# VITA-Group/SinNeRF

Hardware: NVIDIA H100
Metric: rays/sec (64c+64f samples, 8x256 MLP) (higher is better)
Workload: dtype fp32-parity: fp16 hi/lo split x3 on wgmma, fp32 accumulate

## Files before the change

### sinnerf_b200/csrc/field_tc.cu

```cuda
#include <stddef.h>
#include <stdlib.h>

#include <type_traits>
#include <utility>

#include "act16.cuh"
#include "common.cuh"
#include "wgmma.cuh"

namespace snb {
using namespace wg;

constexpr int kTile = 128;
constexpr int kNh = 128;
constexpr int kKc = 32;
constexpr uint32_t kStepBytes = kNh * 16 * 2;
constexpr int kWgs = 2;
constexpr int kThreads = (kWgs + 1) * 128;
constexpr int kProducerRegs = 24, kConsumerRegs = 240;
static_assert(128 * kProducerRegs + kWgs * 128 * kConsumerRegs <= 65536, "register file");
constexpr size_t kSmemOptIn = 232448;

enum { SRC_ENC = 0, SRC_HID = 1, SRC_DIR = 2 };

// ... 243 lines not shown
    double acc = k == kWidth ? (double)bd[n] : 0.0;
    for (int j = 0; j < kWidth; ++j) acc += (double)Wd[n * 283 + j] * (double)(k == kWidth ? bf[j] : Wf[j * kWidth + k]);
    if (k == kWidth) fused[kHalf * kWidth + n] = (float)acc;
    else fused[n * kWidth + k] = (float)acc;
  }
}

template <bool kBf16, bool kSplit>
__global__ void pack_tc_kernel(ParamPtrs pp, int precision, int new_activation, unsigned char* image, int only_if_dirty) {
  constexpr ConstLayout CL = make_const_layout();
  const ChunkTable& tab = c_chunks;
  PackedHeader* hdr = reinterpret_cast<PackedHeader*>(image);
  if (only_if_dirty && !hdr->dirty) return;
  float* cst = reinterpret_cast<float*>(image + sizeof(PackedHeader));
  unsigned char* chunks = image + sizeof(PackedHeader) + kConstBytes;
  const float* fused = reinterpret_cast<const float*>(chunks + chunks_bytes(precision));
  const int gtid = blockIdx.x * blockDim.x + threadIdx.x, gsz = gridDim.x * blockDim.x;
  if (gtid == 0) {
    hdr->magic = kMagic;
    hdr->precision = precision;
    hdr->new_activation = new_activation;
    hdr->cta_group = 1;
  }
  for (int e = gtid; e < kConstFloats; e += gsz) {
    float v = 0.f;
    if (e < CL.sigma_w) {
      int l = 0;
      while (l + 1 < kNumGemm && e >= CL.b[l + 1]) ++l;
      v = l == 9 ? fused[kHalf * kWidth + (e - CL.b[l])] : pp.p[param_weight_index(l) + 1][e - CL.b[l]];
    } else if (e < CL.sigma_b) v = pp.p[kSigmaW][e - CL.sigma_w];
    else if (e == CL.sigma_b) v = pp.p[kSigmaB][0];
    else if (e >= CL.rgb_w && e < CL.rgb_b) v = pp.p[kRgbW][e - CL.rgb_w];
    else if (e >= CL.rgb_b && e < CL.rgb_b + 3) v = pp.p[kRgbB][e - CL.rgb_b];
    cst[e] = v;
  }
  constexpr int kParts = kSplit ? 2 : 1;
  const int total = tab.steps_total * kNh * 16;
  for (int e = gtid; e < total; e += gsz) {
    const int gstep = e / (kNh * 16), rem = e - gstep * (kNh * 16);
    const int r = rem >> 4, k16 = rem & 15;
    int ci = 0;
    while (ci + 1 < tab.n_total && gstep >= tab.c[ci + 1].off) ++ci;
    const Chunk c = tab.c[ci];
    const int kk = (gstep - c.off) * 16 + k16;
    const int l = c.layer;
    const int n = c.half * kNh + r;
    const int kpad = c.w16 * 16 + kk;
    const int col = kpad < gemm_k(l) ? gemm_src_col(l, kpad) : -1;
    const int src_k = l == 0 ? 63 : (l == 4 ? 319 : (l == 9 ? 283 : 256));
    float w = col >= 0 ? pp.p[param_weight_index(l)][n * src_k + col] : 0.f;
    if (l == 9 && kpad < kWidth) w = fused[n * kWidth + kpad];
    const uint32_t part = kStepBytes * c.steps;
    unsigned char* base = chunks + (size_t)c.off * (kStepBytes * kParts);
    const uint32_t off = (uint32_t)(kk >> 3) * (kNh * 16) + r * 16 + (kk & 7) * 2;
    if (kSplit) {
      uint16_t hi, lo;
      split16<kBf16>(w, hi, lo);
      *reinterpret_cast<uint16_t*>(base + off) = hi;
      *reinterpret_cast<uint16_t*>(base + part + off) = lo;
    } else {
      if (!kBf16) w = fminf(fmaxf(w, -65504.f), 65504.f);
      *reinterpret_cast<uint16_t*>(base + off) = cvt16<kBf16>(w);
    }
  }
}

int launch_pack_tc(const float* const* params, int precision, int new_activation, void* image, int only_if_dirty,
                   cudaStream_t st) {
  ParamPtrs pp;
  for (int i = 0; i < SNB_N_PARAM_TENSORS; ++i) pp.p[i] = params[i];
  unsigned char* img = reinterpret_cast<unsigned char*>(image);
  if (precision < SNB_PREC_F16X3 || precision > SNB_PREC_F16)
    return fail(SNB_ERR_INVALID, "launch_pack_tc: precision %d is not a tensor-core mode", precision);
  float* fused = reinterpret_cast<float*>(img + sizeof(PackedHeader) + kConstBytes + chunks_bytes(precision));
  fuse_bottleneck_kernel<<<132, 256, 0, st>>>(pp, fused, reinterpret_cast<const PackedHeader*>(img), only_if_dirty);
  if (int rc = check_launch("fuse_bottleneck_kernel")) return rc;
  if (precision == SNB_PREC_F16X3) pack_tc_kernel<false, true><<<264, 256, 0, st>>>(pp, precision, new_activation, img, only_if_dirty);
  else if (precision == SNB_PREC_BF16X3) pack_tc_kernel<true, true><<<264, 256, 0, st>>>(pp, precision, new_activation, img, only_if_dirty);
  else if (precision == SNB_PREC_BF16) pack_tc_kernel<true, false><<<264, 256, 0, st>>>(pp, precision, new_activation, img, only_if_dirty);
  else pack_tc_kernel<false, false><<<264, 256, 0, st>>>(pp, precision, new_activation, img, only_if_dirty);
  return check_launch("pack_tc_kernel");
}

template <bool kSplit>
struct TcSmem {
  static constexpr int kParts = kSplit ? 2 : 1;
  static constexpr uint32_t kStageBytes = kStepBytes * (kKc / 16) * kParts;
  static constexpr size_t kActBytes = (size_t)kParts * kTile * (kWidth + kXyzPad) * 2;
  static constexpr int kStages = (int)((kSmemOptIn - 128 - kActBytes) / (kStageBytes + 2 * sizeof(uint64_t)));
  alignas(128) unsigned char ring[kStages][kStageBytes];
  alignas(128) unsigned char hid[kParts][kTile * kWidth * 2];
  alignas(128) unsigned char enc[kParts][kTile * kXyzPad * 2];
  uint64_t full[kStages], empty[kStages];
};
static_assert(kDirPad <= kXyzPad, "the direction encoding fits in the xyz encoding's buffer");
static_assert(sizeof(TcSmem<true>) + 128 <= kSmemOptIn && sizeof(TcSmem<false>) + 128 <= kSmemOptIn, "shared memory");
static_assert(TcSmem<true>::kStages >= 4 && TcSmem<false>::kStages >= 6, "weight ring depth");

struct TcParams {
  const unsigned char* image;
  const float* rays;
  const float* z;
  int n_samples;
  const float* x;
  long long x_stride;
  long long n_points;
  int sigma_only;
  float* out;
  float* save_enc;
  float* save_dir;
  float* save_h;
  float* save_g;
  unsigned char* a_enc;
  unsigned char* a_dir;
  unsigned char* a_h;
  unsigned char* a_g;
  uint32_t* a_mask;
  long long ppad;
};

template <bool kBf16, bool kSplit, bool kEmbedded, int kTrain = 0>
__global__ void __launch_bounds__(kThreads, 1) field_tc_kernel(TcParams p) {
  static_assert(!(kTrain != 0 && kEmbedded), "the training forward is the fused (rays, z) entry only");
  using Smem = TcSmem<kSplit>;
  extern __shared__ unsigned char smem_raw[];
  Smem& s = *reinterpret_cast<Smem*>((reinterpret_cast<uintptr_t>(smem_raw) + 127) & ~uintptr_t(127));
  constexpr ConstLayout CL = make_const_layout();
  constexpr int kStages = Smem::kStages;
  constexpr int kParts = Smem::kParts;
  const ChunkTable& tab = c_chunks;
  const int tid = threadIdx.x, warp = tid >> 5, lane = tid & 31;
  const PackedHeader* hdr = reinterpret_cast<const PackedHeader*>(p.image);
  const int new_activation = hdr->new_activation;
  const float* g_cst = reinterpret_cast<const float*>(p.image + sizeof(PackedHeader));
  const unsigned char* g_chunks = p.image + sizeof(PackedHeader) + kConstBytes;
  const long long ntiles = (p.n_points + kTile - 1) / kTile;
  const int n_chunks = p.sigma_only ? tab.n_sigma_only : tab.n_total;

  if (tid == 0) {
    for (int i = 0; i < kStages; ++i) { mbar_init(&s.full[i], 1); mbar_init(&s.empty[i], kWgs * 4); }
    fence_mbar_init();
  }
  __syncthreads();

  if (warp >= kWgs * 4) {
    setmaxnreg_dec<kProducerRegs>();
    if (warp == kWgs * 4 && elect_one()) {
      const long long my_tiles = ntiles > (long long)blockIdx.x ? (ntiles - 1 - blockIdx.x) / gridDim.x + 1 : 0;
      const long long n_loads = my_tiles * n_chunks;
      uint32_t st = 0, ph = 0;
      int ci = 0;
      for (long long i = 0; i < n_loads; ++i) {
        mbar_wait(&s.empty[st], ph ^ 1);
        const Chunk c = tab.c[ci];
        const uint32_t bytes = kStepBytes * kParts * c.steps;
        mbar_arrive_expect_tx(&s.full[st], bytes);
        bulk_g2s(s.ring[st], g_chunks + (size_t)c.off * (kStepBytes * kParts), bytes, &s.full[st]);
        if (++ci == n_chunks) ci = 0;
        if (++st == kStages) { st = 0; ph ^= 1; }
      }
    }
    return;
  }
  setmaxnreg_inc<kConsumerRegs>();

  const int wgi = warp >> 2, wq = warp & 3, tq = lane & 3;
  const int r0 = wgi * 64 + wq * 16 + (lane >> 2);
  auto wg_sync = [&]() { named_bar_sync(1 + wgi, 128); };
  constexpr uint32_t kHidPart = kTile * kWidth * 2, kEncPart = kTile * kXyzPad * 2;
  constexpr uint32_t kOffRing = offsetof(Smem, ring), kOffHid = offsetof(Smem, hid), kOffEnc = offsetof(Smem, enc);
  const uint32_t sbase = smem_u32(&s);
  const uint32_t a_wg = sbase + wgi * 64 * 16;
  const uint32_t hid_thr = sbase + kOffHid + r0 * 16 + tq * 4;
  const int er = wgi * 64 + (tid & 63), epart = (tid >> 6) & 1;

  auto store_cell16 = [&](unsigned char* base, long long pt, int f8, int F, const float (&v)[8]) SNB_INLINE {
    if (pt >= p.ppad) return;
    const bool live = pt < p.n_points;
    uint4 c;
    c.x = live ? pack_half2_sat(v[0], v[1]) : 0u; c.y = live ? pack_half2_sat(v[2], v[3]) : 0u;
    c.z = live ? pack_half2_sat(v[4], v[5]) : 0u; c.w = live ? pack_half2_sat(v[6], v[7]) : 0u;
    *reinterpret_cast<uint4*>(base + a16_cell(pt, f8, F)) = c;
  };

  struct RowIn { float4 q0, q1; float z; };
  RowIn in{};
  auto load_row = [&](long long tile) SNB_INLINE {
    const long long pt = tile * kTile + er;
    if (!kEmbedded && tile < ntiles && pt < p.n_points) {
      const long long ray = pt / p.n_samples;
      in.q0 = *reinterpret_cast<const float4*>(p.rays + ray * 8);
      in.q1 = *reinterpret_cast<const float4*>(p.rays + ray * 8 + 4);
      in.z = p.z[pt];
    }
  };
  auto encode = [&](auto ltag, auto ptag, long long tile) SNB_INLINE {
    constexpr int L = decltype(ltag)::value, P = decltype(ptag)::value;
    constexpr bool kXyz = L == SNB_XYZ_FREQS;
    constexpr int kCh = 3 * (2 * L + 1), kPad = (kCh + 7) / 8 * 8, kK8 = kPad / 16;
    constexpr int c_lo = 8 * kK8 * P, c_hi = 8 * kK8 * (P + 1);
    const long long pt = tile * kTile + er;
    const bool live = pt < p.n_points;
    float v[kPad];
#pragma unroll
    for (int j = 0; j < kPad; ++j) v[j] = 0.f;
    if (kEmbedded) {
      const float* xr = p.x + pt * p.x_stride;
      const int nin = p.sigma_only ? kXyzCh : kXyzCh + kDirCh;
#pragma unroll
      for (int j = c_lo; j < (c_hi < kCh ? c_hi : kCh); ++j) {
        const int col = kXyz ? j : kXyzCh + j;
        v[j] = (live && col < nin) ? xr[col] : 0.f;
      }
    } else {
      float x[3] = {0.f, 0.f, 0.f};
      if (live) {
        if (kXyz) {
          x[0] = __fadd_rn(in.q0.x, __fmul_rn(in.q0.w, in.z));
          x[1] = __fadd_rn(in.q0.y, __fmul_rn(in.q1.x, in.z));
          x[2] = __fadd_rn(in.q0.z, __fmul_rn(in.q1.y, in.z));
        } else {
          x[0] = in.q0.w; x[1] = in.q1.x; x[2] = in.q1.y;
        }
      }
      v[0] = x[0]; v[1] = x[1]; v[2] = x[2];
#pragma unroll
      for (int f = 0; f < L; ++f)
#pragma unroll
        for (int c = 0; c < 3; ++c) {
          const int cs = 3 + 6 * f + c, cc = cs + 3;
          if ((cs >= c_lo && cs < c_hi) || (cc >= c_lo && cc < c_hi)) {
            float sn, cs_;
            if (kSplit) sincosf(x[c] * (float)(1 << f), &sn, &cs_);
            else sincos_fast(x[c] * (float)(1 << f), &sn, &cs_);
            v[cs] = sn;
            v[cc] = cs_;
          }
        }
    }
    static_for<kK8>([&](auto ktag) SNB_INLINE {
      constexpr int k8 = kK8 * P + decltype(ktag)::value;
      const float v8[8] = {v[8 * k8], v[8 * k8 + 1], v[8 * k8 + 2], v[8 * k8 + 3], v[8 * k8 + 4], v[8 * k8 + 5], v[8 * k8 + 6], v[8 * k8 + 7]};
      if (!kEmbedded) {
        if (kTrain == 1 && live) {
          float4* dst = reinterpret_cast<float4*>((kXyz ? p.save_enc + pt * kXyzPad : p.save_dir + pt * kDirPad) + k8 * 8);
          dst[0] = make_float4(v8[0], v8[1], v8[2], v8[3]); dst[1] = make_float4(v8[4], v8[5], v8[6], v8[7]);
        }
        if (kTrain == 2) store_cell16(kXyz ? p.a_enc : p.a_dir, pt, k8, kXyz ? kXyzPad : kDirPad, v8);
      }
      uint32_t h[4], l[4];
#pragma unroll
      for (int j = 0; j < 4; ++j) split_pair<kBf16, kSplit>(v8[2 * j], v8[2 * j + 1], h[j], l[j]);
      const uint32_t a = sbase + kOffEnc + k8 * (kTile * 16) + er * 16;
      st_shared_v4(a, h[0], h[1], h[2], h[3]);
      if (kSplit) st_shared_v4(a + kEncPart, l[0], l[1], l[2], l[3]);
    });
  };
  auto encode_rows = [&](auto ltag, long long tile) SNB_INLINE {
    if (epart == 0) encode(ltag, std::integral_constant<int, 0>{}, tile);
    else encode(ltag, std::integral_constant<int, 1>{}, tile);
  };

  auto mma = [&](float (&d)[64], uint64_t a, uint64_t b, bool first) SNB_INLINE {
    if (first) {
      if (kBf16) wgmma_m64n128_bf16_first(d, a, b);
      else wgmma_m64n128_f16_first(d, a, b);
    } else {
      if (kBf16) wgmma_m64n128_bf16(d, a, b, 1u);
      else wgmma_m64n128_f16(d, a, b, 1u);
    }
  };
  auto issue_step = [&](float (&d)[64], uint32_t ah, uint32_t al, uint32_t bh, uint32_t bl, bool first) SNB_INLINE {
    const uint64_t da_h = make_smem_desc(ah, kTile * 16, 128), db_h = make_smem_desc(bh, kNh * 16, 128);
    mma(d, da_h, db_h, first);
    if (kSplit) {
      mma(d, make_smem_desc(al, kTile * 16, 128), db_h, false);
      mma(d, da_h, make_smem_desc(bl, kNh * 16, 128), false);
    }
  };

  constexpr bool kDrained = kTrain != 0;
  float acc[2][64];
  float sig[2] = {0.f, 0.f};

  uint32_t st = 0, ph = 0;
  auto prev_stage = [&]() { return st == 0 ? (uint32_t)kStages - 1 : st - 1; };
  auto issue = [&](auto ctag) SNB_INLINE {
    constexpr int ci = decltype(ctag)::value;
    constexpr Chunk c = h_chunks.c[ci];
    float (&d)[64] = acc[c.half];
    mbar_wait(&s.full[st], ph);
    wgmma_fence();
    const uint32_t bh = sbase + kOffRing + st * Smem::kStageBytes, bl = bh + kStepBytes * c.steps;
    uint32_t abase;
    asm volatile("mov.b32 %0, %1;" : "=r"(abase) : "r"(a_wg));
    const uint32_t ah = abase + (c.src == SRC_HID ? kOffHid : kOffEnc) + c.a16 * 2 * (kTile * 16);
    constexpr uint32_t part = c.src == SRC_HID ? kHidPart : kEncPart;
    static_for<c.steps>([&](auto ktag) SNB_INLINE {
      constexpr int ks = decltype(ktag)::value;
      issue_step(d, ah + ks * 2 * (kTile * 16), ah + ks * 2 * (kTile * 16) + part, bh + ks * kStepBytes,
                 bl + ks * kStepBytes, ks == 0 && c.first);
    });
    wgmma_commit();
    if (kDrained ? !(c.first && c.half == 0) : ci != 0) {
      wgmma_wait<1>();
      if (lane == 0) mbar_arrive(&s.empty[prev_stage()]);
      __syncwarp();
    }
    if (++st == kStages) { st = 0; ph ^= 1; }
  };
  auto issue_range = [&](auto c0tag, auto ntag) SNB_INLINE {
    static_for<decltype(ntag)::value>([&](auto i) SNB_INLINE { issue(Int<decltype(c0tag)::value + decltype(i)::value>{}); });
  };
  auto drain = [&]() {
    wgmma_wait<0>();
    if (lane == 0) mbar_arrive(&s.empty[prev_stage()]);
    __syncwarp();
  };

  struct Block16 { uint32_t h16[4][2], mask[2]; };
  auto epi_block = [&](auto sigtag, auto htag, auto btag, int l, long long pt0) SNB_INLINE {
    constexpr bool kSigma = decltype(sigtag)::value;
    constexpr int h = decltype(htag)::value, b = decltype(btag)::value;
    const float* bias = g_cst + l * kWidth;
    const float (&d)[64] = acc[h];
    Block16 k16{};
    if (kSigma && h == 0 && b == 0) { sig[0] = 0.f; sig[1] = 0.f; }
    static_for<4>([&](auto jtag) SNB_INLINE {
      constexpr int jj = decltype(jtag)::value, j = 4 * b + jj;
      const int col = h * kNh + 8 * j + 2 * tq;
      const float2 bb = ldg_f2_here(bias + col);
#pragma unroll
      for (int rr = 0; rr < 2; ++rr) {
        float x0 = d[4 * j + 2 * rr] + bb.x, x1 = d[4 * j + 2 * rr + 1] + bb.y;
        uint32_t hi, lo;
        if (kTrain == 0 && !kSigma) {
          split_pair_relu<kBf16, kSplit>(x0, x1, hi, lo);
        } else {
          x0 = fmaxf(x0, 0.f); x1 = fmaxf(x1, 0.f);
          if (kSigma) {
            const float2 ww = ldg_f2_here(g_cst + CL.sigma_w + col);
            sig[rr] = fmaf(x0, ww.x, sig[rr]); sig[rr] = fmaf(x1, ww.y, sig[rr]);
          }
          split_pair<kBf16, kSplit, true>(x0, x1, hi, lo);
          const long long pt = pt0 + 8 * rr;
          if (kTrain == 1 && pt < p.n_points)
            *reinterpret_cast<float2*>(p.save_h + ((size_t)l * p.n_points + pt) * kWidth + col) = make_float2(x0, x1);
          if (kTrain == 2) {
            k16.h16[jj][rr] = kBf16 ? pack_half2_sat(x0, x1) : hi;
            k16.mask[rr] |= ((x0 > 0.f ? 1u : 0u) << (col & 31)) | ((x1 > 0.f ? 1u : 0u) << ((col & 31) + 1));
          }
        }
        const uint32_t a = hid_thr + (h * 16 + j) * (kTile * 16) + rr * 128;
        st_shared_u32(a, hi);
        if (kSplit) st_shared_u32(a + kHidPart, lo);
      }
    });
    if (kTrain == 2) {
#pragma unroll
      for (int rr = 0; rr < 2; ++rr) {
        k16.mask[rr] |= __shfl_xor_sync(0xffffffffu, k16.mask[rr], 1);
        k16.mask[rr] |= __shfl_xor_sync(0xffffffffu, k16.mask[rr], 2);
      }
    }
    return k16;
  };
  auto epi_half_end = [&]() SNB_INLINE {
    fence_proxy_async_smem();
    wg_sync();
  };
  auto sigma_head = [&](long long pt0) SNB_INLINE {
#pragma unroll
    for (int rr = 0; rr < 2; ++rr) {
      float v = sig[rr];
      v += __shfl_xor_sync(0xffffffffu, v, 1);
      v += __shfl_xor_sync(0xffffffffu, v, 2);
      sig[rr] = v + __ldg(g_cst + CL.sigma_b);
      const long long pt = pt0 + 8 * rr;
      if (p.sigma_only && tq == 0 && pt < p.n_points) p.out[pt] = sig[rr];
    }
  };

  auto dir_epilogue = [&](const float (&d)[64], long long pt0) SNB_INLINE {
    const float sh = new_activation ? 1.0f : 0.0f;
    float a[2][3] = {{0.f, 0.f, 0.f}, {0.f, 0.f, 0.f}};
#pragma unroll
    for (int j = 0; j < 16; ++j) {
      const int col = 8 * j + 2 * tq;
      const float2 bb = __ldg(reinterpret_cast<const float2*>(g_cst + CL.b[9] + col));
      const float2 w0 = __ldg(reinterpret_cast<const float2*>(g_cst + CL.rgb_w + col));
      const float2 w1 = __ldg(reinterpret_cast<const float2*>(g_cst + CL.rgb_w + kHalf + col));
      const float2 w2 = __ldg(reinterpret_cast<const float2*>(g_cst + CL.rgb_w + 2 * kHalf + col));
#pragma unroll
      for (int rr = 0; rr < 2; ++rr) {
        const long long pt = pt0 + 8 * rr;
        float x0 = d[4 * j + 2 * rr] + (bb.x - sh), x1 = d[4 * j + 2 * rr + 1] + (bb.y - sh);
        if (new_activation) { x0 = softplus_fast(x0); x1 = softplus_fast(x1); }
        else { x0 = fmaxf(x0, 0.f); x1 = fmaxf(x1, 0.f); }
        if (kTrain == 1 && pt < p.n_points) *reinterpret_cast<float2*>(p.save_g + pt * kHalf + col) = make_float2(x0, x1);
        if (kTrain == 2 && pt < p.ppad)
          *reinterpret_cast<uint32_t*>(p.a_g + a16_cell(pt, col >> 3, kHalf) + (col & 7) * 2) =
              pt < p.n_points ? pack_half2_sat(x0, x1) : 0u;
        a[rr][0] = fmaf(x1, w0.y, fmaf(x0, w0.x, a[rr][0]));
        a[rr][1] = fmaf(x1, w1.y, fmaf(x0, w1.x, a[rr][1]));
        a[rr][2] = fmaf(x1, w2.y, fmaf(x0, w2.x, a[rr][2]));
      }
    }
#pragma unroll
    for (int rr = 0; rr < 2; ++rr) {
      float c[3];
#pragma unroll
      for (int k = 0; k < 3; ++k) {
        float v = a[rr][k];
        v += __shfl_xor_sync(0xffffffffu, v, 1);
        v += __shfl_xor_sync(0xffffffffu, v, 2);
        v += __ldg(g_cst + CL.rgb_b + k);
        c[k] = new_activation ? widened_sigmoid_f(v) : sigmoid_f(v);
      }
      const long long pt = pt0 + 8 * rr;
      if (tq == 0 && pt < p.n_points) reinterpret_cast<float4*>(p.out)[pt] = make_float4(c[0], c[1], c[2], sig[rr]);
    }
  };

  auto trunk_epilogue = [&](auto ltag, int l, long long tile, long long pt0) SNB_INLINE {
    constexpr int L = decltype(ltag)::value;
    Block16 k16[2][4];
    static_for<2>([&](auto htag) SNB_INLINE {
      static_for<4>([&](auto btag) SNB_INLINE {
        k16[decltype(htag)::value][decltype(btag)::value] = epi_block(std::bool_constant<L == 7>{}, htag, btag, l, pt0);
      });
    });
    if (L == 7) sigma_head(pt0);
    if (L == 4 && !p.sigma_only) encode_rows(Int<SNB_DIR_FREQS>{}, tile);
    epi_half_end();
    if (kTrain == 2) {
      unsigned char* hb = p.a_h + (size_t)l * (size_t)p.ppad * (kWidth * 2);
#pragma unroll
      for (int rr = 0; rr < 2; ++rr) {
        const long long pt = pt0 + 8 * rr;
        if (pt >= p.ppad) continue;
        const bool live = pt < p.n_points;
#pragma unroll
        for (int h = 0; h < 2; ++h) {
#pragma unroll
          for (int j = 0; j < 16; ++j) {
            const int col = h * kNh + 8 * j + 2 * tq;
            *reinterpret_cast<uint32_t*>(hb + a16_cell(pt, col >> 3, kWidth) + (col & 7) * 2) =
                live ? k16[h][j / 4].h16[j % 4][rr] : 0u;
          }
#pragma unroll
          for (int b = 0; b < 4; ++b)
            if (tq == 0) p.a_mask[a16_mask_index(l, h * 4 + b, pt, p.ppad)] = live ? k16[h][b].mask[rr] : 0u;
        }
      }
    }
  };

  auto trunk_layer = [&](auto ltag, int l, long long tile, long long pt0) SNB_INLINE {
    constexpr int L = decltype(ltag)::value;
    constexpr int c0 = chunk_index(L, 0), n0 = chunk_count(L, 0), c1 = chunk_index(L, 1), n1 = chunk_count(L, 1);
    constexpr int e = enc_chunks(L);
    if constexpr (kDrained) {
      issue_range(Int<c0>{}, Int<n0>{});
      issue_range(Int<c1>{}, Int<n1>{});
      drain();
      trunk_epilogue(ltag, l, tile, pt0);
    } else if constexpr (L == 0) {
      issue_range(Int<c0>{}, Int<n0>{});
      static_for<4>([&](auto btag) SNB_INLINE {
        constexpr int b = decltype(btag)::value;
        if constexpr (b < n1) issue(Int<c1 + b>{});
        epi_block(std::false_type{}, Int<0>{}, btag, 0, pt0);
      });
      epi_half_end();
      wgmma_wait<0>();
    } else {
      static_for<4>([&](auto btag) SNB_INLINE {
        issue(Int<c0 + decltype(btag)::value>{});
        epi_block(std::false_type{}, Int<1>{}, btag, l - 1, pt0);
      });
      epi_half_end();
      issue_range(Int<c0 + 4>{}, Int<n0 - 4>{});
      issue_range(Int<c1>{}, Int<e + 1>{});
      static_for<4>([&](auto btag) SNB_INLINE {
        issue(Int<c1 + e + 1 + decltype(btag)::value>{});
        epi_block(std::bool_constant<L == 7>{}, Int<0>{}, btag, l, pt0);
      });
      if (L == 4 && !p.sigma_only) encode_rows(Int<SNB_DIR_FREQS>{}, tile);
      epi_half_end();
      issue_range(Int<c1 + e + 5>{}, Int<n1 - e - 5>{});
      if constexpr (L != 7) wgmma_wait<0>();
    }
  };
  auto tile_end = [&](long long tile, long long pt0) SNB_INLINE {
    constexpr int c9 = chunk_index(9, 0), n9 = chunk_count(9, 0);
    load_row(tile + gridDim.x);
    if (p.sigma_only) {
      if constexpr (!kDrained) {
        drain();
        static_for<4>([&](auto btag) SNB_INLINE { epi_block(std::true_type{}, Int<1>{}, btag, 7, pt0); });
        sigma_head(pt0);
        epi_half_end();
      }
      return;
    }
    if constexpr (kDrained) {
      issue_range(Int<c9>{}, Int<n9>{});
    } else {
      static_for<4>([&](auto btag) SNB_INLINE {
        issue(Int<c9 + decltype(btag)::value>{});
        epi_block(std::true_type{}, Int<1>{}, btag, 7, pt0);
      });
      sigma_head(pt0);
      epi_half_end();
      issue_range(Int<c9 + 4>{}, Int<n9 - 4>{});
    }
    drain();
    dir_epilogue(acc[0], pt0);
  };

  load_row(blockIdx.x);
  for (long long tile = blockIdx.x; tile < ntiles; tile += gridDim.x) {
    const long long pt0 = tile * kTile + r0;
    encode_rows(Int<SNB_XYZ_FREQS>{}, tile);
    fence_proxy_async_smem();
    wg_sync();
    trunk_layer(Int<0>{}, 0, tile, pt0);
#pragma unroll 1
    for (int l = 1; l < 4; ++l) trunk_layer(Int<1>{}, l, tile, pt0);
    trunk_layer(Int<4>{}, 4, tile, pt0);
#pragma unroll 1
    for (int l = 5; l < 7; ++l) trunk_layer(Int<1>{}, l, tile, pt0);
    trunk_layer(Int<7>{}, 7, tile, pt0);
    tile_end(tile, pt0);
  }
}

template <bool kBf16, bool kSplit, bool kEmbedded, int kTrain = 0>
static int launch_tc(const TcParams& p, cudaStream_t st) {
  static SmemOptIn optin;
  const long long ntiles = (p.n_points + kTile - 1) / kTile;
  if (ntiles == 0) return SNB_OK;
  const size_t smem = sizeof(TcSmem<kSplit>) + 128;
  auto kern = field_tc_kernel<kBf16, kSplit, kEmbedded, kTrain>;
  if (int rc = ensure_smem(kern, optin, (int)smem, "field_tc")) return rc;
  long long ctas = sm_count();
  if (ctas > ntiles) ctas = ntiles;
  kern<<<(unsigned)ctas, kThreads, smem, st>>>(p);
  return check_launch("field_tc_kernel");
}

template <bool kEmbedded, int kTrain = 0>
static int dispatch_tc(int precision, const TcParams& p, cudaStream_t st) {
  switch (precision) {
    case SNB_PREC_F16X3: return launch_tc<false, true, kEmbedded, kTrain>(p, st);
    case SNB_PREC_BF16X3: return launch_tc<true, true, kEmbedded, kTrain>(p, st);
    case SNB_PREC_BF16: return launch_tc<true, false, kEmbedded, kTrain>(p, st);
    case SNB_PREC_F16: return launch_tc<false, false, kEmbedded, kTrain>(p, st);
  }
  return fail(SNB_ERR_INVALID, "precision %d is not a tensor-core mode", precision);
}

int field_forward_tc(const void* packed, int precision, const float* rays, const float* z, int64_t n_rays,
                     int n_samples, int sigma_only, float* raw, cudaStream_t st) {
  TcParams p{};
  p.image = reinterpret_cast<const unsigned char*>(packed);
  p.rays = rays; p.z = z; p.n_samples = n_samples;
  p.n_points = (long long)n_rays * n_samples;
  p.sigma_only = sigma_only;
  p.out = raw;
  return dispatch_tc<false>(precision, p, st);
}

int field_forward_train_tc(const void* packed, int precision, const float* rays, const float* z, int64_t n_rays,
                           int n_samples, int sigma_only, float* raw, float* save_enc, float* save_dir, float* save_h,
                           float* save_g, cudaStream_t st) {
  TcParams p{};
  p.image = reinterpret_cast<const unsigned char*>(packed);
  p.rays = rays; p.z = z; p.n_samples = n_samples;
  p.n_points = (long long)n_rays * n_samples;
  p.sigma_only = sigma_only;
  p.out = raw;
  p.save_enc = save_enc; p.save_dir = save_dir; p.save_h = save_h; p.save_g = save_g;
  return dispatch_tc<false, 1>(precision, p, st);
}

int field_forward_train16_tc(const void* packed, int precision, const float* rays, const float* z, int64_t n_rays,
                             int n_samples, int sigma_only, float* raw, void* act16, cudaStream_t st) {
  TcParams p{};
  p.image = reinterpret_cast<const unsigned char*>(packed);
  p.rays = rays; p.z = z; p.n_samples = n_samples;
  p.n_points = (long long)n_rays * n_samples;
  p.sigma_only = sigma_only;
  p.out = raw;
  const Act16Layout L = make_act16_layout(p.n_points);
  unsigned char* b = reinterpret_cast<unsigned char*>(act16);
  p.a_enc = b + L.enc; p.a_dir = b + L.dir; p.a_h = b + L.h[0]; p.a_g = b + L.g;
  p.a_mask = reinterpret_cast<uint32_t*>(b + L.mask);
  p.ppad = a16_pad(p.n_points);
  return dispatch_tc<false, 2>(precision, p, st);
}

int mlp_forward_tc(const void* packed, int precision, const float* x, int64_t x_stride, int64_t n_points,
                   int sigma_only, float* out, cudaStream_t st) {
  TcParams p{};
  p.image = reinterpret_cast<const unsigned char*>(packed);
  p.x = x; p.x_stride = x_stride;
  p.n_points = n_points;
  p.sigma_only = sigma_only;
  p.out = out;
  return dispatch_tc<true>(precision, p, st);
}

}
```

### sinnerf_b200/csrc/wgmma.cuh

```cuda
#pragma once
#include <cuda_fp16.h>
#include <cuda_bf16.h>
#include <stdint.h>

namespace snb {
namespace wg {

__device__ __forceinline__ uint32_t smem_u32(const void* p) { return (uint32_t)__cvta_generic_to_shared(p); }

__device__ __forceinline__ bool elect_one() {
  uint32_t pred = 0;
  asm volatile(
      "{\n\t.reg .pred p;\n\t"
      "elect.sync _|p, 0xffffffff;\n\t"
      "selp.u32 %0, 1, 0, p;\n\t}"
      : "=r"(pred));
  return pred != 0;
}

__device__ __forceinline__ void mbar_init(uint64_t* bar, uint32_t count) {
  asm volatile("mbarrier.init.shared::cta.b64 [%0], %1;" ::"r"(smem_u32(bar)), "r"(count));
}
__device__ __forceinline__ void fence_mbar_init() { asm volatile("fence.mbarrier_init.release.cluster;" ::: "memory"); }
__device__ __forceinline__ void mbar_arrive(uint64_t* bar) {
// ... 120 lines not shown
      "{%0, %1, %2, %3, %4, %5, %6, %7, %8, %9, %10, %11, %12, %13, %14, %15, %16, %17, %18, %19, %20, %21, %22, %23, %24, %25, %26, %27, %28, %29, %30, %31, %32, %33, %34, %35, %36, %37, %38, %39, %40, %41, %42, %43, %44, %45, %46, %47, %48, %49, %50, %51, %52, %53, %54, %55, %56, %57, %58, %59, %60, %61, %62, %63}, %64, %65, p, 1, 1, 1, 1;\n\t}"
      : "+f"(d[0]), "+f"(d[1]), "+f"(d[2]), "+f"(d[3]), "+f"(d[4]), "+f"(d[5]), "+f"(d[6]), "+f"(d[7]), "+f"(d[8]), "+f"(d[9]), "+f"(d[10]), "+f"(d[11]), "+f"(d[12]), "+f"(d[13]), "+f"(d[14]), "+f"(d[15]), "+f"(d[16]), "+f"(d[17]), "+f"(d[18]), "+f"(d[19]), "+f"(d[20]), "+f"(d[21]), "+f"(d[22]), "+f"(d[23]), "+f"(d[24]), "+f"(d[25]), "+f"(d[26]), "+f"(d[27]), "+f"(d[28]), "+f"(d[29]), "+f"(d[30]), "+f"(d[31]), "+f"(d[32]), "+f"(d[33]), "+f"(d[34]), "+f"(d[35]), "+f"(d[36]), "+f"(d[37]), "+f"(d[38]), "+f"(d[39]), "+f"(d[40]), "+f"(d[41]), "+f"(d[42]), "+f"(d[43]), "+f"(d[44]), "+f"(d[45]), "+f"(d[46]), "+f"(d[47]), "+f"(d[48]), "+f"(d[49]), "+f"(d[50]), "+f"(d[51]), "+f"(d[52]), "+f"(d[53]), "+f"(d[54]), "+f"(d[55]), "+f"(d[56]), "+f"(d[57]), "+f"(d[58]), "+f"(d[59]), "+f"(d[60]), "+f"(d[61]), "+f"(d[62]), "+f"(d[63])
      : "l"(a_desc), "l"(b_desc), "r"(accumulate)
      : "memory");
}

__device__ __forceinline__ void wgmma_m64n64_f16_mn(float (&d)[32], uint64_t a_desc, uint64_t b_desc, uint32_t accumulate) {
  asm volatile(
      "{\n\t.reg .pred p;\n\t"
      "setp.ne.b32 p, %34, 0;\n\t"
      "wgmma.mma_async.sync.aligned.m64n64k16.f32.f16.f16 "
      "{%0, %1, %2, %3, %4, %5, %6, %7, %8, %9, %10, %11, %12, %13, %14, %15, %16, %17, %18, %19, %20, %21, %22, %23, %24, %25, %26, %27, %28, %29, %30, %31}, %32, %33, p, 1, 1, 1, 1;\n\t}"
      : "+f"(d[0]), "+f"(d[1]), "+f"(d[2]), "+f"(d[3]), "+f"(d[4]), "+f"(d[5]), "+f"(d[6]), "+f"(d[7]), "+f"(d[8]), "+f"(d[9]), "+f"(d[10]), "+f"(d[11]), "+f"(d[12]), "+f"(d[13]), "+f"(d[14]), "+f"(d[15]), "+f"(d[16]), "+f"(d[17]), "+f"(d[18]), "+f"(d[19]), "+f"(d[20]), "+f"(d[21]), "+f"(d[22]), "+f"(d[23]), "+f"(d[24]), "+f"(d[25]), "+f"(d[26]), "+f"(d[27]), "+f"(d[28]), "+f"(d[29]), "+f"(d[30]), "+f"(d[31])
      : "l"(a_desc), "l"(b_desc), "r"(accumulate)
      : "memory");
}

__device__ __forceinline__ void wgmma_m64n32_f16_mn(float (&d)[16], uint64_t a_desc, uint64_t b_desc, uint32_t accumulate) {
  asm volatile(
      "{\n\t.reg .pred p;\n\t"
      "setp.ne.b32 p, %18, 0;\n\t"
      "wgmma.mma_async.sync.aligned.m64n32k16.f32.f16.f16 "
      "{%0, %1, %2, %3, %4, %5, %6, %7, %8, %9, %10, %11, %12, %13, %14, %15}, %16, %17, p, 1, 1, 1, 1;\n\t}"
      : "+f"(d[0]), "+f"(d[1]), "+f"(d[2]), "+f"(d[3]), "+f"(d[4]), "+f"(d[5]), "+f"(d[6]), "+f"(d[7]), "+f"(d[8]), "+f"(d[9]), "+f"(d[10]), "+f"(d[11]), "+f"(d[12]), "+f"(d[13]), "+f"(d[14]), "+f"(d[15])
      : "l"(a_desc), "l"(b_desc), "r"(accumulate)
      : "memory");
}

__device__ __forceinline__ void wgmma_m64n128_f16_rs(float (&d)[64], const uint32_t (&a)[4], uint64_t b_desc, uint32_t accumulate) {
  asm volatile(
      "{\n\t.reg .pred p;\n\t"
      "setp.ne.b32 p, %69, 0;\n\t"
      "wgmma.mma_async.sync.aligned.m64n128k16.f32.f16.f16 "
      "{%0, %1, %2, %3, %4, %5, %6, %7, %8, %9, %10, %11, %12, %13, %14, %15, %16, %17, %18, %19, %20, %21, %22, %23, %24, %25, %26, %27, %28, %29, %30, %31, %32, %33, %34, %35, %36, %37, %38, %39, %40, %41, %42, %43, %44, %45, %46, %47, %48, %49, %50, %51, %52, %53, %54, %55, %56, %57, %58, %59, %60, %61, %62, %63}, {%64, %65, %66, %67}, %68, p, 1, 1, 0;\n\t}"
      : "+f"(d[0]), "+f"(d[1]), "+f"(d[2]), "+f"(d[3]), "+f"(d[4]), "+f"(d[5]), "+f"(d[6]), "+f"(d[7]), "+f"(d[8]), "+f"(d[9]), "+f"(d[10]), "+f"(d[11]), "+f"(d[12]), "+f"(d[13]), "+f"(d[14]), "+f"(d[15]), "+f"(d[16]), "+f"(d[17]), "+f"(d[18]), "+f"(d[19]), "+f"(d[20]), "+f"(d[21]), "+f"(d[22]), "+f"(d[23]), "+f"(d[24]), "+f"(d[25]), "+f"(d[26]), "+f"(d[27]), "+f"(d[28]), "+f"(d[29]), "+f"(d[30]), "+f"(d[31]), "+f"(d[32]), "+f"(d[33]), "+f"(d[34]), "+f"(d[35]), "+f"(d[36]), "+f"(d[37]), "+f"(d[38]), "+f"(d[39]), "+f"(d[40]), "+f"(d[41]), "+f"(d[42]), "+f"(d[43]), "+f"(d[44]), "+f"(d[45]), "+f"(d[46]), "+f"(d[47]), "+f"(d[48]), "+f"(d[49]), "+f"(d[50]), "+f"(d[51]), "+f"(d[52]), "+f"(d[53]), "+f"(d[54]), "+f"(d[55]), "+f"(d[56]), "+f"(d[57]), "+f"(d[58]), "+f"(d[59]), "+f"(d[60]), "+f"(d[61]), "+f"(d[62]), "+f"(d[63])
      : "r"(a[0]), "r"(a[1]), "r"(a[2]), "r"(a[3]), "l"(b_desc), "r"(accumulate)
      : "memory");
}

__device__ __forceinline__ void wgmma_m64n256_bf16_mn(float (&d)[128], uint64_t a_desc, uint64_t b_desc, uint32_t accumulate) {
  asm volatile(
      "{\n\t.reg .pred p;\n\t"
      "setp.ne.b32 p, %130, 0;\n\t"
      "wgmma.mma_async.sync.aligned.m64n256k16.f32.bf16.bf16 "
      "{%0, %1, %2, %3, %4, %5, %6, %7, %8, %9, %10, %11, %12, %13, %14, %15, %16, %17, %18, %19, %20, %21, %22, %23, %24, %25, %26, %27, %28, %29, %30, %31, %32, %33, %34, %35, %36, %37, %38, %39, %40, %41, %42, %43, %44, %45, %46, %47, %48, %49, %50, %51, %52, %53, %54, %55, %56, %57, %58, %59, %60, %61, %62, %63, %64, %65, %66, %67, %68, %69, %70, %71, %72, %73, %74, %75, %76, %77, %78, %79, %80, %81, %82, %83, %84, %85, %86, %87, %88, %89, %90, %91, %92, %93, %94, %95, %96, %97, %98, %99, %100, %101, %102, %103, %104, %105, %106, %107, %108, %109, %110, %111, %112, %113, %114, %115, %116, %117, %118, %119, %120, %121, %122, %123, %124, %125, %126, %127}, %128, %129, p, 1, 1, 1, 1;\n\t}"
      : "+f"(d[0]), "+f"(d[1]), "+f"(d[2]), "+f"(d[3]), "+f"(d[4]), "+f"(d[5]), "+f"(d[6]), "+f"(d[7]), "+f"(d[8]), "+f"(d[9]), "+f"(d[10]), "+f"(d[11]), "+f"(d[12]), "+f"(d[13]), "+f"(d[14]), "+f"(d[15]), "+f"(d[16]), "+f"(d[17]), "+f"(d[18]), "+f"(d[19]), "+f"(d[20]), "+f"(d[21]), "+f"(d[22]), "+f"(d[23]), "+f"(d[24]), "+f"(d[25]), "+f"(d[26]), "+f"(d[27]), "+f"(d[28]), "+f"(d[29]), "+f"(d[30]), "+f"(d[31]), "+f"(d[32]), "+f"(d[33]), "+f"(d[34]), "+f"(d[35]), "+f"(d[36]), "+f"(d[37]), "+f"(d[38]), "+f"(d[39]), "+f"(d[40]), "+f"(d[41]), "+f"(d[42]), "+f"(d[43]), "+f"(d[44]), "+f"(d[45]), "+f"(d[46]), "+f"(d[47]), "+f"(d[48]), "+f"(d[49]), "+f"(d[50]), "+f"(d[51]), "+f"(d[52]), "+f"(d[53]), "+f"(d[54]), "+f"(d[55]), "+f"(d[56]), "+f"(d[57]), "+f"(d[58]), "+f"(d[59]), "+f"(d[60]), "+f"(d[61]), "+f"(d[62]), "+f"(d[63]), "+f"(d[64]), "+f"(d[65]), "+f"(d[66]), "+f"(d[67]), "+f"(d[68]), "+f"(d[69]), "+f"(d[70]), "+f"(d[71]), "+f"(d[72]), "+f"(d[73]), "+f"(d[74]), "+f"(d[75]), "+f"(d[76]), "+f"(d[77]), "+f"(d[78]), "+f"(d[79]), "+f"(d[80]), "+f"(d[81]), "+f"(d[82]), "+f"(d[83]), "+f"(d[84]), "+f"(d[85]), "+f"(d[86]), "+f"(d[87]), "+f"(d[88]), "+f"(d[89]), "+f"(d[90]), "+f"(d[91]), "+f"(d[92]), "+f"(d[93]), "+f"(d[94]), "+f"(d[95]), "+f"(d[96]), "+f"(d[97]), "+f"(d[98]), "+f"(d[99]), "+f"(d[100]), "+f"(d[101]), "+f"(d[102]), "+f"(d[103]), "+f"(d[104]), "+f"(d[105]), "+f"(d[106]), "+f"(d[107]), "+f"(d[108]), "+f"(d[109]), "+f"(d[110]), "+f"(d[111]), "+f"(d[112]), "+f"(d[113]), "+f"(d[114]), "+f"(d[115]), "+f"(d[116]), "+f"(d[117]), "+f"(d[118]), "+f"(d[119]), "+f"(d[120]), "+f"(d[121]), "+f"(d[122]), "+f"(d[123]), "+f"(d[124]), "+f"(d[125]), "+f"(d[126]), "+f"(d[127])
      : "l"(a_desc), "l"(b_desc), "r"(accumulate)
      : "memory");
}

__device__ __forceinline__ void wgmma_m64n64_bf16_mn(float (&d)[32], uint64_t a_desc, uint64_t b_desc, uint32_t accumulate) {
  asm volatile(
      "{\n\t.reg .pred p;\n\t"
      "setp.ne.b32 p, %34, 0;\n\t"
      "wgmma.mma_async.sync.aligned.m64n64k16.f32.bf16.bf16 "
      "{%0, %1, %2, %3, %4, %5, %6, %7, %8, %9, %10, %11, %12, %13, %14, %15, %16, %17, %18, %19, %20, %21, %22, %23, %24, %25, %26, %27, %28, %29, %30, %31}, %32, %33, p, 1, 1, 1, 1;\n\t}"
      : "+f"(d[0]), "+f"(d[1]), "+f"(d[2]), "+f"(d[3]), "+f"(d[4]), "+f"(d[5]), "+f"(d[6]), "+f"(d[7]), "+f"(d[8]), "+f"(d[9]), "+f"(d[10]), "+f"(d[11]), "+f"(d[12]), "+f"(d[13]), "+f"(d[14]), "+f"(d[15]), "+f"(d[16]), "+f"(d[17]), "+f"(d[18]), "+f"(d[19]), "+f"(d[20]), "+f"(d[21]), "+f"(d[22]), "+f"(d[23]), "+f"(d[24]), "+f"(d[25]), "+f"(d[26]), "+f"(d[27]), "+f"(d[28]), "+f"(d[29]), "+f"(d[30]), "+f"(d[31])
      : "l"(a_desc), "l"(b_desc), "r"(accumulate)
      : "memory");
}

__device__ __forceinline__ void wgmma_m64n32_bf16_mn(float (&d)[16], uint64_t a_desc, uint64_t b_desc, uint32_t accumulate) {
  asm volatile(
      "{\n\t.reg .pred p;\n\t"
      "setp.ne.b32 p, %18, 0;\n\t"
      "wgmma.mma_async.sync.aligned.m64n32k16.f32.bf16.bf16 "
      "{%0, %1, %2, %3, %4, %5, %6, %7, %8, %9, %10, %11, %12, %13, %14, %15}, %16, %17, p, 1, 1, 1, 1;\n\t}"
      : "+f"(d[0]), "+f"(d[1]), "+f"(d[2]), "+f"(d[3]), "+f"(d[4]), "+f"(d[5]), "+f"(d[6]), "+f"(d[7]), "+f"(d[8]), "+f"(d[9]), "+f"(d[10]), "+f"(d[11]), "+f"(d[12]), "+f"(d[13]), "+f"(d[14]), "+f"(d[15])
      : "l"(a_desc), "l"(b_desc), "r"(accumulate)
      : "memory");
}

__device__ __forceinline__ void wgmma_m64n128_bf16_rs(float (&d)[64], const uint32_t (&a)[4], uint64_t b_desc, uint32_t accumulate) {
  asm volatile(
      "{\n\t.reg .pred p;\n\t"
      "setp.ne.b32 p, %69, 0;\n\t"
      "wgmma.mma_async.sync.aligned.m64n128k16.f32.bf16.bf16 "
      "{%0, %1, %2, %3, %4, %5, %6, %7, %8, %9, %10, %11, %12, %13, %14, %15, %16, %17, %18, %19, %20, %21, %22, %23, %24, %25, %26, %27, %28, %29, %30, %31, %32, %33, %34, %35, %36, %37, %38, %39, %40, %41, %42, %43, %44, %45, %46, %47, %48, %49, %50, %51, %52, %53, %54, %55, %56, %57, %58, %59, %60, %61, %62, %63}, {%64, %65, %66, %67}, %68, p, 1, 1, 0;\n\t}"
      : "+f"(d[0]), "+f"(d[1]), "+f"(d[2]), "+f"(d[3]), "+f"(d[4]), "+f"(d[5]), "+f"(d[6]), "+f"(d[7]), "+f"(d[8]), "+f"(d[9]), "+f"(d[10]), "+f"(d[11]), "+f"(d[12]), "+f"(d[13]), "+f"(d[14]), "+f"(d[15]), "+f"(d[16]), "+f"(d[17]), "+f"(d[18]), "+f"(d[19]), "+f"(d[20]), "+f"(d[21]), "+f"(d[22]), "+f"(d[23]), "+f"(d[24]), "+f"(d[25]), "+f"(d[26]), "+f"(d[27]), "+f"(d[28]), "+f"(d[29]), "+f"(d[30]), "+f"(d[31]), "+f"(d[32]), "+f"(d[33]), "+f"(d[34]), "+f"(d[35]), "+f"(d[36]), "+f"(d[37]), "+f"(d[38]), "+f"(d[39]), "+f"(d[40]), "+f"(d[41]), "+f"(d[42]), "+f"(d[43]), "+f"(d[44]), "+f"(d[45]), "+f"(d[46]), "+f"(d[47]), "+f"(d[48]), "+f"(d[49]), "+f"(d[50]), "+f"(d[51]), "+f"(d[52]), "+f"(d[53]), "+f"(d[54]), "+f"(d[55]), "+f"(d[56]), "+f"(d[57]), "+f"(d[58]), "+f"(d[59]), "+f"(d[60]), "+f"(d[61]), "+f"(d[62]), "+f"(d[63])
      : "r"(a[0]), "r"(a[1]), "r"(a[2]), "r"(a[3]), "l"(b_desc), "r"(accumulate)
      : "memory");
}

}
}
```

Before: 1.139 million.

## Keep hidden-activation hi fragments in registers and feed wgmma from registers

In the inference path, the hi half of each hidden activation is now kept in registers (ahi[16][4]) and fed to register-sourced wgmma, instead of being written to shared memory. Only the lo part still goes to shared memory. The freed shared memory deepens the weight ring (4 to 8 stages for split mode), and some warpgroup syncs and fences are skipped when hidden data no longer passes through smem. The direction input is reloaded from global memory instead of being held across tiles. The risk is higher register pressure: 64 extra registers per thread on top of two 64-float accumulators, within a 240-register budget, which could cause spills.

```diff
diff --git a/sinnerf_b200/csrc/field_tc.cu b/sinnerf_b200/csrc/field_tc.cu
--- a/sinnerf_b200/csrc/field_tc.cu
+++ b/sinnerf_b200/csrc/field_tc.cu
@@ -349,20 +349,26 @@
   return check_launch("pack_tc_kernel");
 }
 
-template <bool kSplit>
+template <bool kSplit, bool kHiRegs>
 struct TcSmem {
   static constexpr int kParts = kSplit ? 2 : 1;
+  static constexpr int kHidParts = kHiRegs ? kParts - 1 : kParts;
   static constexpr uint32_t kStageBytes = kStepBytes * (kKc / 16) * kParts;
-  static constexpr size_t kActBytes = (size_t)kParts * kTile * (kWidth + kXyzPad) * 2;
+  static constexpr size_t kHidBytes = kHidParts ? (size_t)kHidParts * kTile * kWidth * 2 : 128;
+  static constexpr size_t kActBytes = kHidBytes + (size_t)kParts * kTile * kXyzPad * 2;
   static constexpr int kStages = (int)((kSmemOptIn - 128 - kActBytes) / (kStageBytes + 2 * sizeof(uint64_t)));
   alignas(128) unsigned char ring[kStages][kStageBytes];
-  alignas(128) unsigned char hid[kParts][kTile * kWidth * 2];
+  alignas(128) unsigned char hid[kHidBytes];
   alignas(128) unsigned char enc[kParts][kTile * kXyzPad * 2];
   uint64_t full[kStages], empty[kStages];
 };
+__host__ __device__ constexpr bool hi_in_regs(int train) { return train == 0; }
 static_assert(kDirPad <= kXyzPad, "the direction encoding fits in the xyz encoding's buffer");
-static_assert(sizeof(TcSmem<true>) + 128 <= kSmemOptIn && sizeof(TcSmem<false>) + 128 <= kSmemOptIn, "shared memory");
-static_assert(TcSmem<true>::kStages >= 4 && TcSmem<false>::kStages >= 6, "weight ring depth");
+static_assert(sizeof(TcSmem<true, false>) + 128 <= kSmemOptIn && sizeof(TcSmem<false, false>) + 128 <= kSmemOptIn &&
+              sizeof(TcSmem<true, true>) + 128 <= kSmemOptIn && sizeof(TcSmem<false, true>) + 128 <= kSmemOptIn,
+              "shared memory");
+static_assert(TcSmem<true, false>::kStages == 4 && TcSmem<false, false>::kStages == 18 &&
+              TcSmem<true, true>::kStages == 8 && TcSmem<false, true>::kStages == 26, "weight ring depth");
 
 struct TcParams {
   const unsigned char* image;
@@ -389,7 +395,8 @@
 template <bool kBf16, bool kSplit, bool kEmbedded, int kTrain = 0>
 __global__ void __launch_bounds__(kThreads, 1) field_tc_kernel(TcParams p) {
   static_assert(!(kTrain != 0 && kEmbedded), "the training forward is the fused (rays, z) entry only");
-  using Smem = TcSmem<kSplit>;
+  using Smem = TcSmem<kSplit, hi_in_regs(kTrain)>;
+  constexpr bool kHiRegs = hi_in_regs(kTrain);
   extern __shared__ unsigned char smem_raw[];
   Smem& s = *reinterpret_cast<Smem*>((reinterpret_cast<uintptr_t>(smem_raw) + 127) & ~uintptr_t(127));
   constexpr ConstLayout CL = make_const_layout();
@@ -435,6 +442,7 @@
   const int r0 = wgi * 64 + wq * 16 + (lane >> 2);
   auto wg_sync = [&]() { named_bar_sync(1 + wgi, 128); };
   constexpr uint32_t kHidPart = kTile * kWidth * 2, kEncPart = kTile * kXyzPad * 2;
+  constexpr uint32_t kHidLo = kHiRegs ? 0u : kHidPart;
   constexpr uint32_t kOffRing = offsetof(Smem, ring), kOffHid = offsetof(Smem, hid), kOffEnc = offsetof(Smem, enc);
   const uint32_t sbase = smem_u32(&s);
   const uint32_t a_wg = sbase + wgi * 64 * 16;
@@ -454,6 +462,7 @@
   RowIn in{};
   auto load_row = [&](long long tile) SNB_INLINE {
     const long long pt = tile * kTile + er;
+    if constexpr (kHiRegs) in = RowIn{};
     if (!kEmbedded && tile < ntiles && pt < p.n_points) {
       const long long ray = pt / p.n_samples;
       in.q0 = *reinterpret_cast<const float4*>(p.rays + ray * 8);
@@ -486,6 +495,9 @@
           x[0] = __fadd_rn(in.q0.x, __fmul_rn(in.q0.w, in.z));
           x[1] = __fadd_rn(in.q0.y, __fmul_rn(in.q1.x, in.z));
           x[2] = __fadd_rn(in.q0.z, __fmul_rn(in.q1.y, in.z));
+        } else if constexpr (kHiRegs) {
+          const float* d = p.rays + (pt / p.n_samples) * 8 + 3;
+          x[0] = d[0]; x[1] = d[1]; x[2] = d[2];
         } else {
           x[0] = in.q0.w; x[1] = in.q1.x; x[2] = in.q1.y;
         }
@@ -537,6 +549,15 @@
       else wgmma_m64n128_f16(d, a, b, 1u);
     }
   };
+  auto mma_rs = [&](float (&d)[64], const uint32_t (&a)[4], uint64_t b, bool first) SNB_INLINE {
+    if (first) {
+      if (kBf16) wgmma_m64n128_bf16_rs_first(d, a, b);
+      else wgmma_m64n128_f16_rs_first(d, a, b);
+    } else {
+      if (kBf16) wgmma_m64n128_bf16_rs(d, a, b, 1u);
+      else wgmma_m64n128_f16_rs(d, a, b, 1u);
+    }
+  };
   auto issue_step = [&](float (&d)[64], uint32_t ah, uint32_t al, uint32_t bh, uint32_t bl, bool first) SNB_INLINE {
     const uint64_t da_h = make_smem_desc(ah, kTile * 16, 128), db_h = make_smem_desc(bh, kNh * 16, 128);
     mma(d, da_h, db_h, first);
@@ -549,6 +570,7 @@
   constexpr bool kDrained = kTrain != 0;
   float acc[2][64];
   float sig[2] = {0.f, 0.f};
+  uint32_t ahi[16][4];
 
   uint32_t st = 0, ph = 0;
   auto prev_stage = [&]() { return st == 0 ? (uint32_t)kStages - 1 : st - 1; };
@@ -562,12 +584,24 @@
     uint32_t abase;
     asm volatile("mov.b32 %0, %1;" : "=r"(abase) : "r"(a_wg));
     const uint32_t ah = abase + (c.src == SRC_HID ? kOffHid : kOffEnc) + c.a16 * 2 * (kTile * 16);
-    constexpr uint32_t part = c.src == SRC_HID ? kHidPart : kEncPart;
-    static_for<c.steps>([&](auto ktag) SNB_INLINE {
-      constexpr int ks = decltype(ktag)::value;
-      issue_step(d, ah + ks * 2 * (kTile * 16), ah + ks * 2 * (kTile * 16) + part, bh + ks * kStepBytes,
-                 bl + ks * kStepBytes, ks == 0 && c.first);
-    });
+    if constexpr (kHiRegs && c.src == SRC_HID) {
+      static_for<c.steps>([&](auto ktag) SNB_INLINE {
+        constexpr int ks = decltype(ktag)::value;
+        const uint64_t db_h = make_smem_desc(bh + ks * kStepBytes, kNh * 16, 128);
+        mma_rs(d, ahi[c.a16 + ks], db_h, ks == 0 && c.first);
+        if (kSplit) {
+          mma(d, make_smem_desc(ah + ks * 2 * (kTile * 16), kTile * 16, 128), db_h, false);
+          mma_rs(d, ahi[c.a16 + ks], make_smem_desc(bl + ks * kStepBytes, kNh * 16, 128), false);
+        }
+      });
+    } else {
+      constexpr uint32_t part = c.src == SRC_HID ? kHidPart : kEncPart;
+      static_for<c.steps>([&](auto ktag) SNB_INLINE {
+        constexpr int ks = decltype(ktag)::value;
+        issue_step(d, ah + ks * 2 * (kTile * 16), ah + ks * 2 * (kTile * 16) + part, bh + ks * kStepBytes,
+                   bl + ks * kStepBytes, ks == 0 && c.first);
+      });
+    }
     wgmma_commit();
     if (kDrained ? !(c.first && c.half == 0) : ci != 0) {
       wgmma_wait<1>();
@@ -619,8 +653,9 @@
           }
         }
         const uint32_t a = hid_thr + (h * 16 + j) * (kTile * 16) + rr * 128;
-        st_shared_u32(a, hi);
-        if (kSplit) st_shared_u32(a + kHidPart, lo);
+        if constexpr (kHiRegs) ahi[8 * h + j / 2][(jj & 1) * 2 + rr] = hi;
+        else st_shared_u32(a, hi);
+        if (kSplit) st_shared_u32(a + kHidLo, lo);
       }
     });
     if (kTrain == 2) {
@@ -632,9 +667,11 @@
     }
     return k16;
   };
-  auto epi_half_end = [&]() SNB_INLINE {
-    fence_proxy_async_smem();
-    wg_sync();
+  auto epi_half_end = [&](auto enctag) SNB_INLINE {
+    if constexpr (kSplit || !kHiRegs || decltype(enctag)::value) {
+      fence_proxy_async_smem();
+      wg_sync();
+    }
   };
   auto sigma_head = [&](long long pt0) SNB_INLINE {
 #pragma unroll
@@ -699,7 +736,7 @@
     });
     if (L == 7) sigma_head(pt0);
     if (L == 4 && !p.sigma_only) encode_rows(Int<SNB_DIR_FREQS>{}, tile);
-    epi_half_end();
+    epi_half_end(std::bool_constant<L == 4>{});
     if (kTrain == 2) {
       unsigned char* hb = p.a_h + (size_t)l * (size_t)p.ppad * (kWidth * 2);
 #pragma unroll
@@ -739,14 +776,14 @@
         if constexpr (b < n1) issue(Int<c1 + b>{});
         epi_block(std::false_type{}, Int<0>{}, btag, 0, pt0);
       });
-      epi_half_end();
+      epi_half_end(std::false_type{});
       wgmma_wait<0>();
     } else {
       static_for<4>([&](auto btag) SNB_INLINE {
         issue(Int<c0 + decltype(btag)::value>{});
         epi_block(std::false_type{}, Int<1>{}, btag, l - 1, pt0);
       });
-      epi_half_end();
+      epi_half_end(std::false_type{});
       issue_range(Int<c0 + 4>{}, Int<n0 - 4>{});
       issue_range(Int<c1>{}, Int<e + 1>{});
       static_for<4>([&](auto btag) SNB_INLINE {
@@ -754,20 +791,21 @@
         epi_block(std::bool_constant<L == 7>{}, Int<0>{}, btag, l, pt0);
       });
       if (L == 4 && !p.sigma_only) encode_rows(Int<SNB_DIR_FREQS>{}, tile);
-      epi_half_end();
+      epi_half_end(std::bool_constant<L == 4>{});
       issue_range(Int<c1 + e + 5>{}, Int<n1 - e - 5>{});
       if constexpr (L != 7) wgmma_wait<0>();
     }
   };
   auto tile_end = [&](long long tile, long long pt0) SNB_INLINE {
     constexpr int c9 = chunk_index(9, 0), n9 = chunk_count(9, 0);
-    load_row(tile + gridDim.x);
+    if constexpr (!kHiRegs) load_row(tile + gridDim.x);
     if (p.sigma_only) {
       if constexpr (!kDrained) {
+        load_row(tile + gridDim.x);
         drain();
         static_for<4>([&](auto btag) SNB_INLINE { epi_block(std::true_type{}, Int<1>{}, btag, 7, pt0); });
         sigma_head(pt0);
-        epi_half_end();
+        epi_half_end(std::false_type{});
       }
       return;
     }
@@ -779,8 +817,9 @@
         epi_block(std::true_type{}, Int<1>{}, btag, 7, pt0);
       });
       sigma_head(pt0);
-      epi_half_end();
+      epi_half_end(std::false_type{});
       issue_range(Int<c9 + 4>{}, Int<n9 - 4>{});
+      load_row(tile + gridDim.x);
     }
     drain();
     dir_epilogue(acc[0], pt0);
@@ -808,7 +847,7 @@
   static SmemOptIn optin;
   const long long ntiles = (p.n_points + kTile - 1) / kTile;
   if (ntiles == 0) return SNB_OK;
-  const size_t smem = sizeof(TcSmem<kSplit>) + 128;
+  const size_t smem = sizeof(TcSmem<kSplit, hi_in_regs(kTrain)>) + 128;
   auto kern = field_tc_kernel<kBf16, kSplit, kEmbedded, kTrain>;
   if (int rc = ensure_smem(kern, optin, (int)smem, "field_tc")) return rc;
   long long ctas = sm_count();
diff --git a/sinnerf_b200/csrc/wgmma.cuh b/sinnerf_b200/csrc/wgmma.cuh
--- a/sinnerf_b200/csrc/wgmma.cuh
+++ b/sinnerf_b200/csrc/wgmma.cuh
@@ -226,5 +226,27 @@
       : "memory");
 }
 
-}
-}
+__device__ __forceinline__ void wgmma_m64n128_f16_rs_first(float (&d)[64], const uint32_t (&a)[4], uint64_t b_desc) {
+  asm volatile(
+      "{\n\t.reg .pred p;\n\t"
+      "setp.ne.b32 p, %69, 0;\n\t"
+      "wgmma.mma_async.sync.aligned.m64n128k16.f32.f16.f16 "
+      "{%0, %1, %2, %3, %4, %5, %6, %7, %8, %9, %10, %11, %12, %13, %14, %15, %16, %17, %18, %19, %20, %21, %22, %23, %24, %25, %26, %27, %28, %29, %30, %31, %32, %33, %34, %35, %36, %37, %38, %39, %40, %41, %42, %43, %44, %45, %46, %47, %48, %49, %50, %51, %52, %53, %54, %55, %56, %57, %58, %59, %60, %61, %62, %63}, {%64, %65, %66, %67}, %68, p, 1, 1, 0;\n\t}"
+      : "=f"(d[0]), "=f"(d[1]), "=f"(d[2]), "=f"(d[3]), "=f"(d[4]), "=f"(d[5]), "=f"(d[6]), "=f"(d[7]), "=f"(d[8]), "=f"(d[9]), "=f"(d[10]), "=f"(d[11]), "=f"(d[12]), "=f"(d[13]), "=f"(d[14]), "=f"(d[15]), "=f"(d[16]), "=f"(d[17]), "=f"(d[18]), "=f"(d[19]), "=f"(d[20]), "=f"(d[21]), "=f"(d[22]), "=f"(d[23]), "=f"(d[24]), "=f"(d[25]), "=f"(d[26]), "=f"(d[27]), "=f"(d[28]), "=f"(d[29]), "=f"(d[30]), "=f"(d[31]), "=f"(d[32]), "=f"(d[33]), "=f"(d[34]), "=f"(d[35]), "=f"(d[36]), "=f"(d[37]), "=f"(d[38]), "=f"(d[39]), "=f"(d[40]), "=f"(d[41]), "=f"(d[42]), "=f"(d[43]), "=f"(d[44]), "=f"(d[45]), "=f"(d[46]), "=f"(d[47]), "=f"(d[48]), "=f"(d[49]), "=f"(d[50]), "=f"(d[51]), "=f"(d[52]), "=f"(d[53]), "=f"(d[54]), "=f"(d[55]), "=f"(d[56]), "=f"(d[57]), "=f"(d[58]), "=f"(d[59]), "=f"(d[60]), "=f"(d[61]), "=f"(d[62]), "=f"(d[63])
+      : "r"(a[0]), "r"(a[1]), "r"(a[2]), "r"(a[3]), "l"(b_desc), "r"(0u)
+      : "memory");
+}
+
+__device__ __forceinline__ void wgmma_m64n128_bf16_rs_first(float (&d)[64], const uint32_t (&a)[4], uint64_t b_desc) {
+  asm volatile(
+      "{\n\t.reg .pred p;\n\t"
+      "setp.ne.b32 p, %69, 0;\n\t"
+      "wgmma.mma_async.sync.aligned.m64n128k16.f32.bf16.bf16 "
+      "{%0, %1, %2, %3, %4, %5, %6, %7, %8, %9, %10, %11, %12, %13, %14, %15, %16, %17, %18, %19, %20, %21, %22, %23, %24, %25, %26, %27, %28, %29, %30, %31, %32, %33, %34, %35, %36, %37, %38, %39, %40, %41, %42, %43, %44, %45, %46, %47, %48, %49, %50, %51, %52, %53, %54, %55, %56, %57, %58, %59, %60, %61, %62, %63}, {%64, %65, %66, %67}, %68, p, 1, 1, 0;\n\t}"
+      : "=f"(d[0]), "=f"(d[1]), "=f"(d[2]), "=f"(d[3]), "=f"(d[4]), "=f"(d[5]), "=f"(d[6]), "=f"(d[7]), "=f"(d[8]), "=f"(d[9]), "=f"(d[10]), "=f"(d[11]), "=f"(d[12]), "=f"(d[13]), "=f"(d[14]), "=f"(d[15]), "=f"(d[16]), "=f"(d[17]), "=f"(d[18]), "=f"(d[19]), "=f"(d[20]), "=f"(d[21]), "=f"(d[22]), "=f"(d[23]), "=f"(d[24]), "=f"(d[25]), "=f"(d[26]), "=f"(d[27]), "=f"(d[28]), "=f"(d[29]), "=f"(d[30]), "=f"(d[31]), "=f"(d[32]), "=f"(d[33]), "=f"(d[34]), "=f"(d[35]), "=f"(d[36]), "=f"(d[37]), "=f"(d[38]), "=f"(d[39]), "=f"(d[40]), "=f"(d[41]), "=f"(d[42]), "=f"(d[43]), "=f"(d[44]), "=f"(d[45]), "=f"(d[46]), "=f"(d[47]), "=f"(d[48]), "=f"(d[49]), "=f"(d[50]), "=f"(d[51]), "=f"(d[52]), "=f"(d[53]), "=f"(d[54]), "=f"(d[55]), "=f"(d[56]), "=f"(d[57]), "=f"(d[58]), "=f"(d[59]), "=f"(d[60]), "=f"(d[61]), "=f"(d[62]), "=f"(d[63])
+      : "r"(a[0]), "r"(a[1]), "r"(a[2]), "r"(a[3]), "l"(b_desc), "r"(0u)
+      : "memory");
+}
+
+}
+}
```

Result: no change. 1.136 million, median of 6 (-0.3%).
